# VinAIResearch/Point-Unet

Measured on AMD Instinct MI355X. Metric: points_per_sec_forward, higher is better.
Workload: dtype f32

## Files before the change

### point-unet_amd/csrc/common.h

```cpp
#pragma once

#include <hip/hip_runtime.h>

#include <cstdarg>
#include <cstdint>
#include <cstdio>
#include <cstring>
#include <map>
#include <string>
#include <vector>

#include "../../include/pointseg.h"
#include "../../include/pointseg_train_ops.h"

namespace ps {

void set_error(const char* fmt, ...);

#define PS_HIP(expr)                                                                                  \
    do {                                                                                              \
        hipError_t _e = (expr);                                                                       \
        if (_e != hipSuccess) {                                                                       \
            ps::set_error("%s failed: %s (%s:%d)", #expr, hipGetErrorString(_e), __FILE__, __LINE__); \
            return PS_EHIP;                                                                           \
// ... 91 lines not shown
    int inv_tile = 4096;
    bool gather_reduce_ordered = true;
    int maxpool_bwd_ordered = 1;
    bool train_act_bf16 = true;
    int train_att_gemm_split = -1;
    bool train_att_gemm = true;
    bool train_att128_fwd_gemm = true;
    bool train_fuse_residual = true;
    bool train_merge_syncbn = true;
    int convbn_max_c = 64;
    int convbn_rect_max = 1 << 30;
    bool wgrad_debug = false;
};
void tuning_from_env(Tuning& t);
}

struct ps_context {
    int device = 0;
    ps::Tuning tune;
    hipStream_t own_stream = nullptr;
    hipStream_t stream = nullptr;
    ps::Arena knn_arena;
    ps::Arena net_arena;
    ps::Arena sample_arena;
    ps::DevBuf stage_in;
    ps::DevBuf stage_out;
    ps::DevBuf red_ws;
    ps::DevBuf wgrad_ws;
    ps::PackCache* pack_cache = nullptr;
    ps::DevBuf ops_ring[4];
    int ops_ring_pos = 0;
    bool att_bf16x3 = true;
    bool regchain_b3 = true;
    bool train_b3 = true;
    bool conv_w_transposed = false;
    bool att_df_accum = false;
    const int32_t* walk_order = nullptr;
    int64_t walk_order_n = 0;
    bool pool_bwd_overwrite = false;
    bool train_bf16 = false;
    bool train_act_bf16 = false;
    bool mid_lds_attr = false;
    size_t chain_lds_attr = 48 * 1024;
    std::map<const void*, size_t> regchain_lds_attr;
    bool deferred = false;
    int32_t* h_flags = nullptr;
    unsigned pending_mask = 0;
    uint64_t builds = 0;
    uint64_t samples = 0;
    uint64_t volume_samples = 0;
    uint64_t flag_serial[8] = {};
    int flag_kind[8] = {};
    int flag_slot = 0;
    int sticky_rc = 0;
    std::string sticky_msg;
    hipEvent_t flag_ev[8] = {};
    std::vector<char> host_ring[8];
    int ring_pos = 0;
    std::vector<char>& ring_next() { ring_pos = (ring_pos + 1) & 7; return host_ring[ring_pos]; }
    int check_deferred();
    int check_flag_slot(int s);
    int defer_status(const void* d_words, size_t bytes, int kind, uint64_t serial);
    struct PinSlot { void* p = nullptr; size_t cap = 0; hipEvent_t ev = nullptr; bool busy = false; };
    PinSlot pin[16];
    int pin_pos = 0;
    int upload_async(void* dst, const void* src, size_t bytes);
// ... 69 lines not shown
```

### point-unet_amd/csrc/context.hip

```cpp
#include "common.h"
#include "kdtree_build.h"

#include <cstdlib>

namespace ps {

static thread_local char g_err[512] = "";

void set_error(const char* fmt, ...)
{
    va_list ap;
    va_start(ap, fmt);
    vsnprintf(g_err, sizeof g_err, fmt, ap);
    va_end(ap);
}

int DevBuf::reserve(size_t bytes)
{
    if (bytes <= cap) return PS_OK;
    if (p) {
        hipError_t e = hipDeviceSynchronize();
        if (e != hipSuccess) {
            set_error("hipDeviceSynchronize failed: %s", hipGetErrorString(e));
            return PS_EHIP;
// ... 188 lines not shown
    flag("PS_TRAIN_MERGE_SYNCBN", t.train_merge_syncbn);
    if (num("PS_CONVBN_MAX_C", v) && v >= 0 && v <= 4096) t.convbn_max_c = (int)v;
    if (num("PS_CONVBN_RECT_MAX", v) && v >= 0) t.convbn_rect_max = v > (double)(1 << 30) ? 1 << 30 : (int)v;
    t.wgrad_debug = std::getenv("PS_WGRAD_DEBUG") != nullptr;
#else
    (void)t;
#endif
}
}

extern "C" {
const char* ps_version(void) { return "pointseg-hip 0.1 gfx950"; }
int ps_abi_version(void) { return PS_ABI_VERSION; }

int ps_create(int device, ps_context** out)
{
    PS_CHECK(out != nullptr, "ps_create: out is NULL");
    int count = 0;
    PS_HIP(hipGetDeviceCount(&count));
    PS_CHECK(device >= 0 && device < count, "ps_create: device %d out of range (%d devices)", device, count);
    PS_HIP(hipSetDevice(device));
    ps_context* c = new ps_context();
    c->device = device;
    hipError_t e = hipStreamCreateWithFlags(&c->own_stream, hipStreamNonBlocking);
    if (e != hipSuccess) {
        delete c;
        ps::set_error("hipStreamCreate failed: %s", hipGetErrorString(e));
        return PS_EHIP;
    }
    c->stream = c->own_stream;
    ps::tuning_from_env(c->tune);
#ifdef PS_TUNING_ENV
    if (const char* v = std::getenv("PS_REGCHAIN_B3")) c->regchain_b3 = std::atof(v) != 0;
#endif
    *out = c;
    return PS_OK;
}

int ps_destroy(ps_context* c)
{
    if (!c) return PS_OK;
    (void)hipSetDevice(c->device);
    (void)hipStreamSynchronize(c->stream);
    c->knn_arena.buf.release();
    c->net_arena.buf.release();
    c->sample_arena.buf.release();
    c->stage_in.release();
    c->stage_out.release();
    c->red_ws.release();
    c->wgrad_ws.release();
    for (auto& b : c->ops_ring) b.release();
    if (c->h_flags) (void)hipHostFree(c->h_flags);
    for (auto& e : c->flag_ev)
        if (e) (void)hipEventDestroy(e);
    for (auto& s : c->pin) {
        if (s.p) (void)hipHostFree(s.p);
        if (s.ev) (void)hipEventDestroy(s.ev);
    }
    for (hipEvent_t e : c->event_pool) (void)hipEventDestroy(e);
    if (c->own_stream) (void)hipStreamDestroy(c->own_stream);
    delete c;
    return PS_OK;
}

int ps_set_stream(ps_context* c, void* hip_stream)
{
// ... 95 lines not shown
```

### point-unet_amd/csrc/debug_hooks.h

```cpp
#ifndef POINTSEG_DEBUG_H
#define POINTSEG_DEBUG_H
#include "../../include/pointseg.h"
#ifdef __cplusplus
extern "C" {
#endif
int ps_debug_knn_host(const float* support, const float* queries, int64_t B, int64_t n_support,
                      int64_t n_queries, int64_t K, int32_t* out_idx);
int ps_debug_kdtree_host(const float* support, int64_t n, int32_t* vind, int32_t* nodes, float* pts,
                         int32_t* root_depth, float* bbox);
int ps_debug_kdtree_device(ps_context* ctx, const float* support, int64_t n, int32_t* vind, int32_t* nodes,
                           float* pts, int32_t* root_depth, float* bbox);
#define PS_DEBUG_KDTREE_STATS 22
int ps_debug_kdtree_device_set(ps_context* ctx, const float* support, const int32_t* n, int64_t T, const int32_t* want_copy, int32_t* vind,
                               int32_t* nodes, float* pts, int32_t* fat, int32_t* root_depth, float* bbox, float* copy, int32_t* stats);
int ps_debug_pack_weights(const float* W, int cin, int cout, int ntb, float* out);
int ps_debug_pack_b3(const float* W, int cin, int cout, uint16_t* out);
int ps_debug_gemm32(ps_context* ctx, int split_bf16, const float* x1, int ld1, int c1, const int32_t* g1, const float* x2, int ld2, int c2,
                    const int32_t* g2, int gm, int gn, const float* W, const float* bias, int64_t R, int cout, int leaky, float* y, int ldy);
int ps_debug_gemm32_plan(ps_context* ctx, int split_bf16, int64_t R, int cin, int cout, int* out4);

typedef struct ps_debug_chain_layer {
    const float* W;
    const float* bias;
    int cin, cout, leaky;
    float* y;
    int ldy;
    const float* extra;
    int ld_extra, c_extra;
    const int32_t* extra_gather;
} ps_debug_chain_layer;
typedef struct ps_debug_chain_desc {
    int n_layers;
    ps_debug_chain_layer layer[4];
    const float* x1; const int32_t* g1; int ld1, c1, g1m, g1n;
    const float* x2; const int32_t* g2; int ld2, c2, g2m, g2n;
    int64_t R;
} ps_debug_chain_desc;
int ps_debug_chain(ps_context* ctx, const ps_debug_chain_desc* d, int form);
int ps_debug_chain_plan(const ps_debug_chain_desc* d, int* out4);
int ps_debug_set_regchain_b3(ps_context* ctx, int on);
int ps_debug_att_stage(ps_randla* net, int level, int stage, int form, const float* xyz, const int32_t* idx, const int32_t* order, const float* fg,
                       int64_t n_total, int64_t n_cloud, float* agg);

int ps_debug_set_tuning(ps_context* ctx, const char* field, double value);
int ps_debug_get_tuning(ps_context* ctx, const char* field, double* value);
int ps_debug_tuning_fields(char* buf, int cap);
int ps_debug_volume_sample_args_size(void);

#ifdef __cplusplus
}
#endif
#endif
```

### point-unet_amd/csrc/debug_hooks.hip

```cpp
#include "common.h"

#include <cstring>
#include <vector>
#include "kdtree_build.h"
#include "kdtree_host.h"
#include "rowgemm.h"
#include "attpool.h"
#include "debug_hooks.h"
#include "randla_net.h"

using namespace ps;

extern "C" int ps_debug_volume_sample_args_size(void) { return (int)sizeof(ps_volume_sample_args); }

extern "C" int ps_debug_pack_weights(const float* W, int cin, int cout, int ntb, float* out)
{
    PS_CHECK(W && out && (ntb == 1 || ntb == 2 || ntb == 4), "ps_debug_pack_weights: bad argument");
    pack_weights(W, cin, cout, ntb, out);
    return PS_OK;
}

extern "C" int ps_debug_pack_b3(const float* W, int cin, int cout, uint16_t* out)
{
    PS_CHECK(W && out && cin > 0 && cin % 32 == 0 && cout > 0 && cout % 32 == 0, "ps_debug_pack_b3: bad argument");
// ... 167 lines not shown
            if (regchain_fits(b.steps, b.n, b.s1, b.s2)) rc = regchain(c, b.steps, b.n, b.s1, b.s2, d->R, nullptr);
            else { set_error("ps_debug_chain: not one of regchain's compiled chain shapes"); rc = PS_EINVAL; }
        } else if (form == 2) {
            if (rowchain_lds_plan(b.steps, b.n, b.s1, b.s2, d->R).form == 2) rc = rowchain_lds(c, b.steps, b.n, b.s1, b.s2, d->R);
            else { set_error("ps_debug_chain: the chain does not fit the LDS-staged kernel (channels above %d, mismatched, or a gathered extra)", kChainMaxC); rc = PS_EINVAL; }
        } else {
            RowSrc in1 = b.s1, in2 = b.s2;
            for (int i = 0; i < b.n && rc == PS_OK; ++i) {
                const ChainStep& st = b.steps[i];
                if (i > 0) {
                    in2 = RowSrc();
                    if (st.extra.x) in2 = st.extra;
                }
                float* out = st.y ? st.y : dev + tmp_off[i];
                const int ldo = st.y ? st.ldy : b.L[i].cout;
                rc = rowgemm(c, b.L[i], in1, in2, d->R, out, ldo);
                in1 = RowSrc();
                in1.x = out; in1.ld = ldo; in1.c = b.L[i].cout;
            }
        }
    }
    (void)hipStreamSynchronize(c->stream);
    (void)hipFree(dev);
    return rc;
}

extern "C" int ps_debug_set_regchain_b3(ps_context* c, int on)
{
    PS_CHECK(c && (on == 0 || on == 1), "ps_debug_set_regchain_b3: bad argument");
    c->regchain_b3 = on != 0;
    return PS_OK;
}

extern "C" int ps_debug_att_stage(ps_randla* net, int level, int stage, int form, const float* xyz, const int32_t* idx, const int32_t* order,
                                  const float* fg, int64_t n_total, int64_t n_cloud, float* agg)
{
    PS_CHECK(net && xyz && idx && fg && agg, "ps_debug_att_stage: NULL argument");
    PS_CHECK(net->have_weights, "ps_debug_att_stage: weights not set");
    PS_CHECK(level >= 0 && level < net->cfg.num_layers && (stage == 1 || stage == 2) && form >= 0 && form <= 3, "ps_debug_att_stage: bad level / stage / form");
    PS_CHECK(n_total >= 0 && n_cloud >= 1 && n_total % n_cloud == 0, "ps_debug_att_stage: n_total must be a whole number of clouds");
    ps_context* c = net->ctx;
    PS_HIP(hipSetDevice(c->device));
    const EncLevel& e = net->enc[level];
    const int d = e.d, h = d / 2;
    const bool use_g = d >= 64;
    AttStage s;
    s.xyz = xyz; s.idx = idx; s.order = order; s.fg = fg; s.lfa1 = &e.lfa1; s.agg = agg;
    s.n_total = n_total; s.n_cloud = n_cloud; s.d = d; s.k = net->cfg.k_n; s.ldf = use_g ? h + d : h;
    s.p32 = e.has_p32 ? &e.p32 : nullptr;
    s.lfa2 = stage == 2 ? &e.lfa2 : nullptr;
    s.wbot = use_g ? (stage == 1 ? &e.bot1 : &e.bot2) : nullptr;
    s.wfull = use_g ? nullptr : (stage == 1 ? &e.full1 : &e.full2);
    int rc = PS_EINVAL;
    if (form == 0) rc = att_pool_stage(c, s);
    else if (form == 1 && att_pool32b_fits(s)) rc = att_pool32b_stage(c, s);
    else if (form == 2 && att_pool32_fits(s)) rc = att_pool32_stage(c, s);
    else if (form == 3) rc = att_pool16_stage(c, s);
    else set_error("ps_debug_att_stage: the level (d = %d, %lld rows) does not fit the 32x32 form %d", d, (long long)n_total, form);
    (void)hipStreamSynchronize(c->stream);
    return rc;
}

static bool is_bool(double v) { return v == 0 || v == 1; }
static bool is_int_in(double v, double lo, double hi) { return v >= lo && v <= hi && v == (double)(int64_t)v; }

#define PS_TUNING_FIELDS(X)                                                \
// ... 176 lines not shown
```

### point-unet_amd/csrc/randla.hip

```cpp
#include "attpool.h"
#include "common.h"
#include "randla_net.h"
#include "rowgemm.h"

#include <memory>

namespace ps {

template <int KN>
__global__ __launch_bounds__(256) void pool_max_kernel(const float* __restrict__ feat, const int32_t* __restrict__ idx, const int32_t* __restrict__ order,
                                                       float* __restrict__ out, int rows_out, int m_cloud, int n_cloud, int K, int c4 ,
                                                       unsigned char* __restrict__ ties )
{
    const int per_xcd = (rows_out + 7) >> 3;
    const int xcd = blockIdx.x & 7;
    const size_t lim = (size_t)min(rows_out, (xcd + 1) * per_xcd) * c4;
    for (size_t t = (size_t)xcd * per_xcd * c4 + (size_t)(blockIdx.x >> 3) * 256 + threadIdx.x; t < lim; t += (size_t)(gridDim.x >> 3) * 256) {
        const int r = (int)(t / c4), q = (int)(t - (size_t)r * c4);
        const int row = order ? (r / m_cloud) * m_cloud + order[r] : r;
        const int base = (row / m_cloud) * n_cloud;
        const int32_t* ix = idx + (size_t)row * K;
        const float4* f4 = reinterpret_cast<const float4*>(feat);
        float4 m;
        if constexpr (KN > 0) {
// ... 422 lines not shown
        d_in = 2 * d;
    }

    {
        Stage st(c, "decoder_0", 1);
        PS_TRY(rowgemm(c, net->decoder0, src(X, d_in, d_in), none, B * n[L], dec0, d_in));
    }
    tap(30, dec0, B * n[L] * d_in);

    const float* up = dec0;
    int up_c = d_in;
    for (int j = 0; j < L; ++j) {
        const int lvl = L - 1 - j;
        const float* skip = lvl == 0 ? encb[0] : poolb[lvl - 1];
        const int skip_c = net->dec[j].cout;
        RowSrc s2 = src(up, up_c, up_c);
        s2.gather = pyr->interp_idx[lvl];
        s2.gm = (int)n[lvl];
        s2.gn = (int)n[lvl + 1];
        char nm[48];
        std::snprintf(nm, sizeof nm, "dec%d", j);
        if (j == L - 1) {
            ChainStep ch[4] = {step(net->dec[j], net->keep_taps ? decb[j] : nullptr, skip_c), step(net->fc1, nullptr, 0), step(net->fc2, nullptr, 0),
                               step(net->fc, logits, cfg.num_classes)};
            const RowSrc s1 = src(skip, skip_c, skip_c);
            if (rowchain_fits(ch, 4, s1, s2)) {
                Stage st(c, "head", 1);
                PS_TRY(rowchain(c, ch, 4, s1, s2, B * n[lvl], &net->chains));
                if (net->keep_taps) tap(40 + j, decb[j], B * n[lvl] * skip_c);
                return PS_OK;
            }
        }
        Stage st(c, nm, 1);
        PS_TRY(rowgemm(c, net->dec[j], src(skip, skip_c, skip_c), s2, B * n[lvl], decb[j], skip_c));
        tap(40 + j, decb[j], B * n[lvl] * skip_c);
        up = decb[j];
        up_c = skip_c;
    }
    {
        Stage st(c, "head", 3);
        PS_TRY(rowgemm(c, net->fc1, src(up, up_c, up_c), none, B * n[0], h1, 64));
        PS_TRY(rowgemm(c, net->fc2, src(h1, 64, 64), none, B * n[0], h2, 32));
        PS_TRY(rowgemm(c, net->fc, src(h2, 32, 32), none, B * n[0], logits, cfg.num_classes));
    }
    return PS_OK;
}

extern "C" int ps_randla_keep_taps(ps_randla* net, int on)
{
    PS_CHECK(net, "ps_randla_keep_taps: net is NULL");
    net->keep_taps = on != 0;
    return PS_OK;
}

extern "C" int ps_randla_tap(ps_randla* net, int which, float* host_out, int64_t count)
{
    PS_CHECK(net && host_out, "ps_randla_tap: NULL argument");
    for (auto& t : net->taps)
        if (t.which == which) {
            PS_CHECK(t.count == count, "ps_randla_tap: tensor %d has %lld floats, caller expects %lld", which, (long long)t.count, (long long)count);
            PS_HIP(hipMemcpyAsync(host_out, t.p, sizeof(float) * (size_t)count, hipMemcpyDeviceToHost, net->ctx->stream));
            PS_HIP(hipStreamSynchronize(net->ctx->stream));
            return PS_OK;
        }
    set_error("ps_randla_tap: no tensor %d (run a forward first; the last decoder step's rows are only kept after ps_randla_keep_taps)", which);
    return PS_EINVAL;
}
// ... 1 lines not shown
```

### point-unet_amd/csrc/regchain.hip

```cpp
#include <algorithm>
#include <type_traits>

#include "b3_ops.h"
#include "mfma_tile.h"
#include "rowgemm.h"

namespace ps {

struct RcLayer {
    const float* wp;
    const float* bias;
    float* y;
    const float* ex;
    int ca, cb;
    int ta, tb;
    int cout, ot;
    int ks, ntb;
    int ldy, ldex, leaky;
    int w_off, b_off;
};
struct RcArgs {
    const float* x1; const int32_t* g1; int ld1, g1m, g1n;
    const float* x2; const int32_t* g2; int ld2, g2m, g2n;
    int n, R;
    RcLayer l[kChainMaxSteps];
    const float* image;
    int image_floats;
};

template <int N_, int A0_, int B0_, int O0_, int B1_ = 0, int O1_ = 0, int B2_ = 0, int O2_ = 0, int B3_ = 0, int O3_ = 0>
struct RcShape {
    static constexpr int N = N_, A0 = A0_;
    static constexpr int B[4] = {B0_, B1_, B2_, B3_};
    static constexpr int O[4] = {O0_, O1_, O2_, O3_};
    static constexpr int A(int l) { return l == 0 ? A0_ : O[l - 1]; }
    static constexpr int IN(int l) { return A(l) + B[l]; }
    static constexpr int maxt()
    {
        int m = 1;
        for (int l = 0; l < N_; ++l) {
            m = IN(l) > m ? IN(l) : m;
            m = O[l] > m ? O[l] : m;
        }
        return m;
    }
};

template <int T0, int NT, int MT>
__device__ __forceinline__ void rc_load(float (&dst)[MT][4], const float* __restrict__ rowp, int c, bool vec, int g)
{
#pragma unroll
    for (int t = 0; t < NT; ++t) {
        const int ch = t * 16 + 4 * g;
        if (vec) {
            float4 v = make_float4(0.f, 0.f, 0.f, 0.f);
            if (t + 1 < NT || ch < c) v = *reinterpret_cast<const float4*>(rowp + ch);
            dst[T0 + t][0] = v.x; dst[T0 + t][1] = v.y; dst[T0 + t][2] = v.z; dst[T0 + t][3] = v.w;
        } else {
#pragma unroll
            for (int q = 0; q < 4; ++q) dst[T0 + t][q] = (t + 1 < NT || ch + q < c) ? rowp[ch + q] : 0.f;
        }
    }
}

struct RcF32 {
    static constexpr int kThreads = 256;
    static constexpr int kPairFloats = 256;
    template <int IT, int OT, int MT>
    static __device__ __forceinline__ void mma(f32x4 (&acc)[OT], const float (&act)[MT][4], const float* wl, int lane)
    {
        const float* w = wl + lane;
#pragma unroll
        for (int t0 = 0; t0 < OT; t0 += 4) {
#pragma unroll
            for (int ti = 0; ti < IT; ++ti)
#pragma unroll
                for (int q = 0; q < 4; ++q)
#pragma unroll
                    for (int to = t0; to < (t0 + 4 < OT ? t0 + 4 : OT); ++to)
                        acc[to] = __builtin_amdgcn_mfma_f32_16x16x4f32(w[((to * IT + ti) * 4 + q) * 64], act[ti][q], acc[to], 0, 0, 0);
            if (t0 + 4 < OT) __builtin_amdgcn_sched_barrier(0);
        }
    }
    static __device__ __forceinline__ void stage(const RcLayer& y, float* dst)
    {
        const int it_n = y.ta + y.tb;
        const int ln = threadIdx.x & 63, q = threadIdx.x >> 6;
        const int i = ln & 15, gg = ln >> 4;
        const int npairs = it_n * y.ot;
// ... 50 lines not shown
                    for (int pl = 0; pl < 3; ++pl) a.p[pl] = w[((to * KP + kp) * 3 + pl) * 64];
                    acc[to] = b3_mfma16_6(a, b[kp], acc[to]);
                }
            if (t0 + 4 < OT) __builtin_amdgcn_sched_barrier(0);
        }
    }
    static __device__ __forceinline__ void stage(const RcLayer& y, float* dst)
    {
        const int kp_n = (y.ta + y.tb) / 2;
        uint4* out = reinterpret_cast<uint4*>(dst + y.w_off);
        for (int s = threadIdx.x; s < y.ot * kp_n * 64; s += kThreads) {
            const int ln = s & 63, slot = s >> 6;
            const int to = slot / kp_n, kp = slot - to * kp_n;
            const int i = ln & 15, gg = ln >> 4;
            const int cblk = to / y.ntb, j = to - cblk * y.ntb;
            float v[8];
#pragma unroll
            for (int e = 0; e < 8; ++e) {
                const int ti = 2 * kp + (e >> 2), q = e & 3;
                int k;
                bool kok;
                if (ti < y.ta) { k = ti * 16 + 4 * gg + q; kok = k < y.ca; }
                else { k = (ti - y.ta) * 16 + 4 * gg + q; kok = k < y.cb; k += y.ca; }
                v[e] = 0.f;
                if (kok && to * 16 + i < y.cout) v[e] = y.wp[(((size_t)cblk * y.ks + (k >> 2)) * 64 + ((k & 3) * 16 + i)) * y.ntb + j];
            }
            const B3Planes p = b3_split8<3>(v);
#pragma unroll
            for (int pl = 0; pl < 3; ++pl) out[(slot * 3 + pl) * 64 + ln] = p.p[pl];
        }
    }
};

template <class S, class P, int L>
__device__ __forceinline__ void rc_layer(const RcArgs& a, float (&act)[S::maxt()][4], const float* lds, int lane, int g, int row, int rr, bool ok)
{
    if constexpr (L < S::N) {
        constexpr int IT = S::IN(L), OT = S::O[L], TA = S::A(L), TB = S::B[L];
        const RcLayer& y = a.l[L];
        if constexpr (L > 0 && TB > 0) {
            const bool ve = (y.cb & 3) == 0 && (y.ldex & 3) == 0 && (reinterpret_cast<uintptr_t>(y.ex) & 15) == 0;
            rc_load<TA, TB>(act, y.ex + (size_t)rr * y.ldex, y.cb, ve, g);
        }
        f32x4 acc[OT];
#pragma unroll
        for (int to = 0; to < OT; ++to) acc[to] = f32x4{0.f, 0.f, 0.f, 0.f};
        if constexpr (L > 0) __builtin_amdgcn_sched_barrier(0);
        P::template mma<IT, OT>(acc, act, lds + y.w_off, lane);
        const bool vy = y.y && (y.cout & 3) == 0 && (y.ldy & 3) == 0 && (reinterpret_cast<uintptr_t>(y.y) & 15) == 0;
#pragma unroll
        for (int to = 0; to < OT; ++to) {
            const int ch = to * 16 + 4 * g;
            const float4 b = *reinterpret_cast<const float4*>(lds + y.b_off + ch);
            float v[4] = {acc[to][0] + b.x, acc[to][1] + b.y, acc[to][2] + b.z, acc[to][3] + b.w};
#pragma unroll
            for (int q = 0; q < 4; ++q) {
                if (y.leaky) v[q] = leaky02(v[q]);
                act[to][q] = v[q];
            }
            if (y.y && ok) {
                float* o = y.y + (size_t)row * y.ldy + ch;
                if (vy) {
                    if (to + 1 < OT || ch < y.cout) *reinterpret_cast<float4*>(o) = make_float4(v[0], v[1], v[2], v[3]);
                } else {
#pragma unroll
                    for (int q = 0; q < 4; ++q)
                        if (to + 1 < OT || ch + q < y.cout) o[q] = v[q];
                }
            }
        }
        rc_layer<S, P, L + 1>(a, act, lds, lane, g, row, rr, ok);
    }
}

template <class P>
__device__ __forceinline__ void rc_stage(const RcArgs& a, float* dst)
{
    for (int l = 0; l < a.n; ++l) {
        const RcLayer& y = a.l[l];
        P::stage(y, dst);
        for (int e = threadIdx.x; e < y.ot * 16; e += P::kThreads) dst[y.b_off + e] = e < y.cout ? y.bias[e] : 0.f;
    }
}

template <class P>
__global__ __launch_bounds__(P::kThreads) void rc_pack_kernel(RcArgs a, float* out) { rc_stage<P>(a, out); }

template <class S, class P>
__global__ __launch_bounds__(P::kThreads) void regchain_kernel(RcArgs a)
{
    extern __shared__ __attribute__((aligned(16))) float rc_lds[];
    constexpr int MT = S::maxt(), WAVES = P::kThreads / 64;
    const int wave = threadIdx.x >> 6, lane = threadIdx.x & 63;
    const int p = lane & 15, g = lane >> 4;
    if (a.image) {
        for (int i = threadIdx.x; i < a.image_floats / 4; i += P::kThreads) reinterpret_cast<float4*>(rc_lds)[i] = reinterpret_cast<const float4*>(a.image)[i];
    } else {
        rc_stage<P>(a, rc_lds);
    }
    __syncthreads();

    const bool v1 = (a.l[0].ca & 3) == 0 && (a.ld1 & 3) == 0 && (reinterpret_cast<uintptr_t>(a.x1) & 15) == 0;
    const bool v2 = (a.l[0].cb & 3) == 0 && (a.ld2 & 3) == 0 && (reinterpret_cast<uintptr_t>(a.x2) & 15) == 0;
    const int stride = gridDim.x * WAVES;
    auto load_inputs = [&](int tile, float (&dst)[MT][4]) {
        const int rr = min(tile * 16 + p, a.R - 1);
        const int s1 = a.g1 ? (a.g1m ? (rr / a.g1m) * a.g1n : 0) + a.g1[rr] : rr;
        rc_load<0, S::A0>(dst, a.x1 + (size_t)s1 * a.ld1, a.l[0].ca, v1, g);
        if constexpr (S::B[0] > 0) {
            const int s2 = a.g2 ? (a.g2m ? (rr / a.g2m) * a.g2n : 0) + a.g2[rr] : rr;
            rc_load<S::A0, S::B[0]>(dst, a.x2 + (size_t)s2 * a.ld2, a.l[0].cb, v2, g);
        }
    };
    int tile = blockIdx.x * WAVES + wave;
    float act[MT][4], nxt[MT][4];
    if (tile * 16 < a.R) load_inputs(tile, nxt);
    for (; tile * 16 < a.R; tile += stride) {
#pragma unroll
        for (int t = 0; t < S::IN(0); ++t)
#pragma unroll
            for (int q = 0; q < 4; ++q) act[t][q] = nxt[t][q];
        if ((tile + stride) * 16 < a.R) load_inputs(tile + stride, nxt);
        const int row = tile * 16 + p;
        rc_layer<S, P, 0>(a, act, rc_lds, lane, g, row, min(row, a.R - 1), row < a.R);
    }
}

static inline int rc_tiles(int c) { return (c + 15) / 16; }

using RcFc0 = RcShape<2, 1, 0, 1, 0, 1>;
using RcEnc0 = RcShape<2, 1, 0, 1, 1, 2>;
using RcOne0 = RcShape<1, 1, 0, 1>;
using RcPair1 = RcShape<2, 2, 0, 2, 0, 4>;
using RcPair1b = RcShape<2, 4, 0, 2, 0, 4>;
using RcEnc1 = RcShape<2, 4, 0, 4, 2, 8>;
using RcPair2 = RcShape<2, 8, 0, 4, 0, 8>;
using RcHead = RcShape<4, 2, 2, 2, 0, 4, 0, 2, 0, 1>;

template <class S>
static bool rc_matches(const RcArgs& a)
{
    if (a.n != S::N) return false;
    for (int l = 0; l < S::N; ++l)
        if (a.l[l].ta != S::A(l) || a.l[l].tb != S::B[l] || a.l[l].ot != S::O[l]) return false;
    return true;
}

template <class S>
constexpr bool rc_even_inputs()
{
    for (int l = 0; l < S::N; ++l)
        if (S::IN(l) & 1) return false;
    return true;
}
template <class S>
constexpr bool kRcSplit = std::is_same<S, RcHead>::value || std::is_same<S, RcEnc1>::value || std::is_same<S, RcPair1>::value ||
                          std::is_same<S, RcPair1b>::value;

static size_t rc_layout(RcArgs& a, int pair_floats)
{
    int off = 0;
    for (int i = 0; i < a.n; ++i) {
        RcLayer& y = a.l[i];
        y.w_off = off; off += y.ot * (y.ta + y.tb) * pair_floats;
        y.b_off = off; off += y.ot * 16;
    }
    return (size_t)off * sizeof(float);
}

static bool rc_build(const ChainStep* steps, int n_steps, const RowSrc& s1, const RowSrc& s2, RcArgs& a, size_t& lds_bytes)
{
    if (n_steps < 1 || n_steps > kChainMaxSteps) return false;
    a = RcArgs{};
    a.x1 = s1.x; a.g1 = s1.gather; a.ld1 = s1.ld; a.g1m = s1.gm; a.g1n = s1.gn;
    a.x2 = s2.x; a.g2 = s2.gather; a.ld2 = s2.ld; a.g2m = s2.gm; a.g2n = s2.gn;
    a.n = n_steps;
    int prev = 0;
    for (int i = 0; i < n_steps; ++i) {
        const PackedLinear* L = steps[i].L;
        if (!L || !L->wp || !L->bias) return false;
        if (steps[i].extra.x && (i == 0 || steps[i].extra.gather)) return false;
        RcLayer& y = a.l[i];
        y.wp = L->wp; y.bias = L->bias; y.y = steps[i].y; y.ldy = steps[i].ldy;
        y.ex = i > 0 ? steps[i].extra.x : nullptr; y.ldex = steps[i].extra.ld;
        y.ca = i == 0 ? s1.c : prev;
        y.cb = i == 0 ? s2.c : (steps[i].extra.x ? steps[i].extra.c : 0);
        if (y.ca + y.cb != L->cin) return false;
        y.ta = rc_tiles(y.ca); y.tb = rc_tiles(y.cb);
        y.cout = L->cout; y.ot = rc_tiles(L->cout);
        y.ks = L->ks; y.ntb = L->ntb; y.leaky = L->leaky;
        prev = L->cout;
    }
    lds_bytes = rc_layout(a, RcF32::kPairFloats);
    return rc_matches<RcFc0>(a) || rc_matches<RcEnc0>(a) || rc_matches<RcOne0>(a) || rc_matches<RcPair1>(a) || rc_matches<RcPair1b>(a) ||
           rc_matches<RcEnc1>(a) || rc_matches<RcPair2>(a) || rc_matches<RcHead>(a);
}

bool regchain_fits(const ChainStep* steps, int n_steps, const RowSrc& s1, const RowSrc& s2)
{
    RcArgs a;
    size_t lds = 0;
    return rc_build(steps, n_steps, s1, s2, a, lds);
}

static int rc_blocks(int64_t R, size_t lds_bytes, int waves)
{
    const int64_t tiles = (R + 15) / 16;
    const int per_cu = std::max(1, std::min(16 / waves, (int)(160 * 1024 / std::max<size_t>(lds_bytes, 1))));
    return (int)std::max<int64_t>(1, std::min<int64_t>((tiles + waves - 1) / waves, 256 * per_cu));
}

ChainPlan regchain_plan(const ChainStep* steps, int n_steps, const RowSrc& s1, const RowSrc& s2, int64_t R)
{
    ChainPlan p;
    RcArgs a;
    if (!rc_build(steps, n_steps, s1, s2, a, p.lds_bytes)) return ChainPlan();
    p.form = 1;
    p.blocks = rc_blocks(R, p.lds_bytes, RcF32::kThreads / 64);
    return p;
}

template <class S, class P>
static int rc_run(ps_context* c, RcArgs& a, ChainCache* cache)
{
    constexpr bool split = std::is_same<P, RcB3>::value;
    const size_t lds_bytes = rc_layout(a, P::kPairFloats);
    if (cache) {
        ChainCache::Entry* hit = nullptr;
        for (auto& e : cache->entries)
            if (e.wp0 == a.l[0].wp && e.wp_last == a.l[a.n - 1].wp && e.n == a.n && e.ca == a.l[0].ca && e.cb == a.l[0].cb && e.split == split) hit = &e;
        if (!hit) {
            cache->entries.emplace_back();
            hit = &cache->entries.back();
            hit->wp0 = a.l[0].wp; hit->wp_last = a.l[a.n - 1].wp; hit->n = a.n; hit->ca = a.l[0].ca; hit->cb = a.l[0].cb; hit->split = split;
            PS_TRY(hit->img.reserve(lds_bytes));
            hipLaunchKernelGGL(rc_pack_kernel<P>, dim3(1), dim3(P::kThreads), 0, c->stream, a, hit->img.as<float>());
            PS_HIP(hipGetLastError());
        }
        a.image = hit->img.as<float>();
        a.image_floats = (int)(lds_bytes / sizeof(float));
    }
    size_t& have = c->regchain_lds_attr[reinterpret_cast<const void*>(regchain_kernel<S, P>)];
    if (lds_bytes > 48 * 1024 && lds_bytes > have) {
        PS_HIP(hipFuncSetAttribute(reinterpret_cast<const void*>(regchain_kernel<S, P>), hipFuncAttributeMaxDynamicSharedMemorySize, (int)lds_bytes));
        have = lds_bytes;
    }
    hipLaunchKernelGGL((regchain_kernel<S, P>), dim3(rc_blocks(a.R, lds_bytes, P::kThreads / 64)), dim3(P::kThreads), lds_bytes, c->stream, a);
    PS_HIP(hipGetLastError());
    return PS_OK;
}

template <class S>
static int rc_route(ps_context* c, RcArgs& a, ChainCache* cache)
{
    if constexpr (kRcSplit<S>) {
        static_assert(rc_even_inputs<S>(), "the split-bf16 policy takes its K axis in pairs of 16-channel tiles");
        if (c->regchain_b3) return rc_run<S, RcB3>(c, a, cache);
    }
    return rc_run<S, RcF32>(c, a, cache);
}

int regchain(ps_context* c, const ChainStep* steps, int n_steps, const RowSrc& s1, const RowSrc& s2, int64_t R, ChainCache* cache)
{
    if (R <= 0) return PS_OK;
    RcArgs a;
    size_t lds_bytes = 0;
    PS_CHECK(rc_build(steps, n_steps, s1, s2, a, lds_bytes), "regchain: not one of the compiled chain shapes");
    PS_CHECK(R < (int64_t)1 << 31, "regchain: too many rows");
    a.R = (int)R;
    if (rc_matches<RcFc0>(a)) return rc_route<RcFc0>(c, a, cache);
    if (rc_matches<RcEnc0>(a)) return rc_route<RcEnc0>(c, a, cache);
    if (rc_matches<RcOne0>(a)) return rc_route<RcOne0>(c, a, cache);
    if (rc_matches<RcPair1>(a)) return rc_route<RcPair1>(c, a, cache);
    if (rc_matches<RcPair1b>(a)) return rc_route<RcPair1b>(c, a, cache);
    if (rc_matches<RcEnc1>(a)) return rc_route<RcEnc1>(c, a, cache);
    if (rc_matches<RcPair2>(a)) return rc_route<RcPair2>(c, a, cache);
    return rc_route<RcHead>(c, a, cache);
}

}
```

### point-unet_amd/csrc/rowgemm.h

```cpp
#pragma once

#include <vector>

#include "common.h"

namespace ps {

struct PackedLinear {
    const float* wp = nullptr;
    const float* wq = nullptr;
    const void* wb = nullptr;
    const float* w32 = nullptr;
    const void* w32b = nullptr;
    const float* bias = nullptr;
    int cin = 0, cout = 0;
    int ks = 0;
    int ntb = 0;
    int cblocks = 0;
    int leaky = 0;
    int accum = 0;
    size_t packed_floats() const { return (size_t)cblocks * ks * 64 * ntb; }
    int nchunks() const { return (cin + 63) / 64; }
    size_t kperm_floats() const { return (size_t)cblocks * nchunks() * 16 * 64 * ntb; }
    size_t bf16_bytes() const { return (size_t)cblocks * nchunks() * 2 * 64 * ntb * 16; }
// ... 17 lines not shown
    int rw = 1, cw = 1, sk = 1, pd = 2;
    int rgroups = 0, cgroups = 0;
};
Gemm32Plan gemm32_plan(const Tuning& tn, int64_t R, int cin, int cout);
Gemm32Plan gemm32b_plan(const Tuning& tn, int64_t R, int cin, int cout);
bool gemm32_fits(const PackedLinear& L, const RowSrc& s1, const RowSrc& s2, int64_t R, int ldy);
int gemm32(ps_context* c, const PackedLinear& L, const RowSrc& s1, const RowSrc& s2, int64_t R, float* y, int ldy);
void pack_p32b(const float* W, int cin, int cout, uint16_t* out);
bool gemm32b_fits(const PackedLinear& L, const RowSrc& s1, const RowSrc& s2, int64_t R, int ldy);
int gemm32b(ps_context* c, const PackedLinear& L, const RowSrc& s1, const RowSrc& s2, int64_t R, float* y, int ldy);

int rowgemm(ps_context* c, const PackedLinear& L, const RowSrc& s1, const RowSrc& s2, int64_t R, float* y, int ldy);

constexpr int kChainMaxC = 96;
constexpr int kChainMaxSteps = 4;
struct ChainStep {
    const PackedLinear* L = nullptr;
    float* y = nullptr;
    int ldy = 0;
    RowSrc extra;
};
bool rowchain_fits(const ChainStep* steps, int n_steps, const RowSrc& s1, const RowSrc& s2);
bool regchain_fits(const ChainStep* steps, int n_steps, const RowSrc& s1, const RowSrc& s2);
struct ChainCache {
    struct Entry { const float* wp0 = nullptr; const float* wp_last = nullptr; int n = 0, ca = 0, cb = 0; bool split = false; DevBuf img; };
    std::vector<Entry> entries;
    void clear()
    {
        for (auto& e : entries) e.img.release();
        entries.clear();
    }
};
int regchain(ps_context* c, const ChainStep* steps, int n_steps, const RowSrc& s1, const RowSrc& s2, int64_t R, ChainCache* cache);
int rowchain_lds(ps_context* c, const ChainStep* steps, int n_steps, const RowSrc& s1, const RowSrc& s2, int64_t R);
struct ChainPlan {
    int form = 0;
    int blocks = 0;
    size_t lds_bytes = 0;
    int fast_in = 0;
};
ChainPlan regchain_plan(const ChainStep* steps, int n_steps, const RowSrc& s1, const RowSrc& s2, int64_t R);
ChainPlan rowchain_lds_plan(const ChainStep* steps, int n_steps, const RowSrc& s1, const RowSrc& s2, int64_t R);
ChainPlan rowchain_plan(const ChainStep* steps, int n_steps, const RowSrc& s1, const RowSrc& s2, int64_t R);
int rowchain(ps_context* c, const ChainStep* steps, int n_steps, const RowSrc& s1, const RowSrc& s2, int64_t R, ChainCache* cache = nullptr);

bool gemm_b3_fits(const Tuning& tn, int64_t R, int64_t K, int64_t N, const float* x, int64_t ldx, bool one_plane);
size_t gemm_b3_plane_bytes(int64_t K, int64_t N);
int gemm_b3(ps_context* c, const float* x, int64_t ldx, const float* w, int64_t sk, int64_t sn, const float* bias, int64_t R, int64_t K, int64_t N, int leaky,
            int accumulate, float* y, int64_t ldy, void* planes, int pack = 1);

}
```

Baseline: 192.6 million.

## Specialize register-chain kernels on compile-time layer facts and route decoder layer

Adds compile-time 'facts' template parameters (leaky mask, store mask, partial-tile mask, vectorized last store) to the register-chain kernel. When runtime arguments match a known configuration, the host launches a variant with no alignment checks or bounds guards, and full tiles are split from a single tail tile. It also adds a one-layer decoder chain shape so the non-final decoder linear layers run through the register-chain path instead of rowgemm. This costs more kernel instantiations and adds dispatch logic that must match the runtime facts exactly.

```diff
diff --git a/point-unet_amd/csrc/common.h b/point-unet_amd/csrc/common.h
--- a/point-unet_amd/csrc/common.h
+++ b/point-unet_amd/csrc/common.h
@@ -147,6 +147,7 @@
     int ops_ring_pos = 0;
     bool att_bf16x3 = true;
     bool regchain_b3 = true;
+    bool regchain_special = true;
     bool train_b3 = true;
     bool conv_w_transposed = false;
     bool att_df_accum = false;
diff --git a/point-unet_amd/csrc/context.hip b/point-unet_amd/csrc/context.hip
--- a/point-unet_amd/csrc/context.hip
+++ b/point-unet_amd/csrc/context.hip
@@ -244,6 +244,7 @@
     ps::tuning_from_env(c->tune);
 #ifdef PS_TUNING_ENV
     if (const char* v = std::getenv("PS_REGCHAIN_B3")) c->regchain_b3 = std::atof(v) != 0;
+    if (const char* v = std::getenv("PS_REGCHAIN_SPECIAL")) c->regchain_special = std::atof(v) != 0;
 #endif
     *out = c;
     return PS_OK;
diff --git a/point-unet_amd/csrc/debug_hooks.h b/point-unet_amd/csrc/debug_hooks.h
--- a/point-unet_amd/csrc/debug_hooks.h
+++ b/point-unet_amd/csrc/debug_hooks.h
@@ -39,6 +39,8 @@
 int ps_debug_chain(ps_context* ctx, const ps_debug_chain_desc* d, int form);
 int ps_debug_chain_plan(const ps_debug_chain_desc* d, int* out4);
 int ps_debug_set_regchain_b3(ps_context* ctx, int on);
+int ps_debug_set_regchain_special(ps_context* ctx, int on);
+int ps_debug_regchain_facts(ps_context* ctx, const ps_debug_chain_desc* d, int* out);
 int ps_debug_att_stage(ps_randla* net, int level, int stage, int form, const float* xyz, const int32_t* idx, const int32_t* order, const float* fg,
                        int64_t n_total, int64_t n_cloud, float* agg);
 
diff --git a/point-unet_amd/csrc/debug_hooks.hip b/point-unet_amd/csrc/debug_hooks.hip
--- a/point-unet_amd/csrc/debug_hooks.hip
+++ b/point-unet_amd/csrc/debug_hooks.hip
@@ -223,6 +223,23 @@
     return PS_OK;
 }
 
+extern "C" int ps_debug_set_regchain_special(ps_context* c, int on)
+{
+    PS_CHECK(c && (on == 0 || on == 1), "ps_debug_set_regchain_special: bad argument");
+    c->regchain_special = on != 0;
+    return PS_OK;
+}
+
+extern "C" int ps_debug_regchain_facts(ps_context* c, const ps_debug_chain_desc* d, int* out)
+{
+    PS_CHECK(c && d && out && d->R >= 1, "ps_debug_regchain_facts: bad argument");
+    static const float nothing = 0.f;
+    ChainBuild b;
+    PS_TRY(chain_describe(d, b, &nothing));
+    out[0] = regchain_special_fits(c, b.steps, b.n, b.s1, b.s2, d->R) ? 1 : 0;
+    return PS_OK;
+}
+
 extern "C" int ps_debug_att_stage(ps_randla* net, int level, int stage, int form, const float* xyz, const int32_t* idx, const int32_t* order,
                                   const float* fg, int64_t n_total, int64_t n_cloud, float* agg)
 {
diff --git a/point-unet_amd/csrc/randla.hip b/point-unet_amd/csrc/randla.hip
--- a/point-unet_amd/csrc/randla.hip
+++ b/point-unet_amd/csrc/randla.hip
@@ -478,7 +478,12 @@
             }
         }
         Stage st(c, nm, 1);
-        PS_TRY(rowgemm(c, net->dec[j], src(skip, skip_c, skip_c), s2, B * n[lvl], decb[j], skip_c));
+        ChainStep one[1] = {step(net->dec[j], decb[j], skip_c)};
+        if (j < L - 1 && regchain_fits(one, 1, src(skip, skip_c, skip_c), s2)) {
+            PS_TRY(rowchain(c, one, 1, src(skip, skip_c, skip_c), s2, B * n[lvl], &net->chains));
+        } else {
+            PS_TRY(rowgemm(c, net->dec[j], src(skip, skip_c, skip_c), s2, B * n[lvl], decb[j], skip_c));
+        }
         tap(40 + j, decb[j], B * n[lvl] * skip_c);
         up = decb[j];
         up_c = skip_c;
diff --git a/point-unet_amd/csrc/regchain.hip b/point-unet_amd/csrc/regchain.hip
--- a/point-unet_amd/csrc/regchain.hip
+++ b/point-unet_amd/csrc/regchain.hip
@@ -46,15 +46,27 @@
     }
 };
 
-template <int T0, int NT, int MT>
+struct RcAny {
+    static constexpr bool kAny = true;
+    static constexpr unsigned kLeaky = 0, kStore = 0, kPart = 0;
+    static constexpr bool kVecLast = false;
+};
+template <unsigned LEAKY, unsigned STORE, unsigned PART, bool VEC_LAST>
+struct RcFacts {
+    static constexpr bool kAny = false;
+    static constexpr unsigned kLeaky = LEAKY, kStore = STORE, kPart = PART;
+    static constexpr bool kVecLast = VEC_LAST;
+};
+
+template <int T0, int NT, int MT, int MODE = 0>
 __device__ __forceinline__ void rc_load(float (&dst)[MT][4], const float* __restrict__ rowp, int c, bool vec, int g)
 {
 #pragma unroll
     for (int t = 0; t < NT; ++t) {
         const int ch = t * 16 + 4 * g;
-        if (vec) {
+        if (MODE != 0 || vec) {
             float4 v = make_float4(0.f, 0.f, 0.f, 0.f);
-            if (t + 1 < NT || ch < c) v = *reinterpret_cast<const float4*>(rowp + ch);
+            if (MODE == 2 || t + 1 < NT || ch < c) v = *reinterpret_cast<const float4*>(rowp + ch);
             dst[T0 + t][0] = v.x; dst[T0 + t][1] = v.y; dst[T0 + t][2] = v.z; dst[T0 + t][3] = v.w;
         } else {
 #pragma unroll
@@ -171,22 +183,30 @@
     }
 };
 
-template <class S, class P, int L>
+template <class S, class P, class F, int L, bool TAIL>
 __device__ __forceinline__ void rc_layer(const RcArgs& a, float (&act)[S::maxt()][4], const float* lds, int lane, int g, int row, int rr, bool ok)
 {
     if constexpr (L < S::N) {
         constexpr int IT = S::IN(L), OT = S::O[L], TA = S::A(L), TB = S::B[L];
         const RcLayer& y = a.l[L];
         if constexpr (L > 0 && TB > 0) {
-            const bool ve = (y.cb & 3) == 0 && (y.ldex & 3) == 0 && (reinterpret_cast<uintptr_t>(y.ex) & 15) == 0;
-            rc_load<TA, TB>(act, y.ex + (size_t)rr * y.ldex, y.cb, ve, g);
+            if constexpr (F::kAny) {
+                const bool ve = (y.cb & 3) == 0 && (y.ldex & 3) == 0 && (reinterpret_cast<uintptr_t>(y.ex) & 15) == 0;
+                rc_load<TA, TB>(act, y.ex + (size_t)rr * y.ldex, y.cb, ve, g);
+            } else {
+                rc_load<TA, TB, S::maxt(), (F::kPart >> (4 + L) & 1) ? 1 : 2>(act, y.ex + (size_t)rr * y.ldex, y.cb, true, g);
+            }
         }
         f32x4 acc[OT];
 #pragma unroll
         for (int to = 0; to < OT; ++to) acc[to] = f32x4{0.f, 0.f, 0.f, 0.f};
         if constexpr (L > 0) __builtin_amdgcn_sched_barrier(0);
         P::template mma<IT, OT>(acc, act, lds + y.w_off, lane);
-        const bool vy = y.y && (y.cout & 3) == 0 && (y.ldy & 3) == 0 && (reinterpret_cast<uintptr_t>(y.y) & 15) == 0;
+        constexpr bool kSpec = !F::kAny, kStored = (F::kStore >> L & 1) != 0, kWhole = kSpec && !(F::kPart >> L & 1);
+        constexpr bool kVecStore = L + 1 < S::N || F::kVecLast;
+        const bool leaky = kSpec ? (F::kLeaky >> L & 1) != 0 : y.leaky != 0;
+        const bool stored = kSpec ? kStored && (!TAIL || ok) : y.y && ok;
+        const bool vy = kSpec ? kVecStore : y.y && (y.cout & 3) == 0 && (y.ldy & 3) == 0 && (reinterpret_cast<uintptr_t>(y.y) & 15) == 0;
 #pragma unroll
         for (int to = 0; to < OT; ++to) {
             const int ch = to * 16 + 4 * g;
@@ -194,21 +214,21 @@
             float v[4] = {acc[to][0] + b.x, acc[to][1] + b.y, acc[to][2] + b.z, acc[to][3] + b.w};
 #pragma unroll
             for (int q = 0; q < 4; ++q) {
-                if (y.leaky) v[q] = leaky02(v[q]);
+                if (leaky) v[q] = leaky02(v[q]);
                 act[to][q] = v[q];
             }
-            if (y.y && ok) {
+            if (stored) {
                 float* o = y.y + (size_t)row * y.ldy + ch;
                 if (vy) {
-                    if (to + 1 < OT || ch < y.cout) *reinterpret_cast<float4*>(o) = make_float4(v[0], v[1], v[2], v[3]);
+                    if (kWhole || to + 1 < OT || ch < y.cout) *reinterpret_cast<float4*>(o) = make_float4(v[0], v[1], v[2], v[3]);
                 } else {
 #pragma unroll
                     for (int q = 0; q < 4; ++q)
-                        if (to + 1 < OT || ch + q < y.cout) o[q] = v[q];
+                        if (kWhole || to + 1 < OT || ch + q < y.cout) o[q] = v[q];
                 }
             }
         }
-        rc_layer<S, P, L + 1>(a, act, lds, lane, g, row, rr, ok);
+        rc_layer<S, P, F, L + 1, TAIL>(a, act, lds, lane, g, row, rr, ok);
     }
 }
 
@@ -225,7 +245,7 @@
 template <class P>
 __global__ __launch_bounds__(P::kThreads) void rc_pack_kernel(RcArgs a, float* out) { rc_stage<P>(a, out); }
 
-template <class S, class P>
+template <class S, class P, class F = RcAny>
 __global__ __launch_bounds__(P::kThreads) void regchain_kernel(RcArgs a)
 {
     extern __shared__ __attribute__((aligned(16))) float rc_lds[];
@@ -239,29 +259,62 @@
     }
     __syncthreads();
 
-    const bool v1 = (a.l[0].ca & 3) == 0 && (a.ld1 & 3) == 0 && (reinterpret_cast<uintptr_t>(a.x1) & 15) == 0;
-    const bool v2 = (a.l[0].cb & 3) == 0 && (a.ld2 & 3) == 0 && (reinterpret_cast<uintptr_t>(a.x2) & 15) == 0;
     const int stride = gridDim.x * WAVES;
-    auto load_inputs = [&](int tile, float (&dst)[MT][4]) {
-        const int rr = min(tile * 16 + p, a.R - 1);
-        const int s1 = a.g1 ? (a.g1m ? (rr / a.g1m) * a.g1n : 0) + a.g1[rr] : rr;
-        rc_load<0, S::A0>(dst, a.x1 + (size_t)s1 * a.ld1, a.l[0].ca, v1, g);
-        if constexpr (S::B[0] > 0) {
-            const int s2 = a.g2 ? (a.g2m ? (rr / a.g2m) * a.g2n : 0) + a.g2[rr] : rr;
-            rc_load<S::A0, S::B[0]>(dst, a.x2 + (size_t)s2 * a.ld2, a.l[0].cb, v2, g);
-        }
-    };
     int tile = blockIdx.x * WAVES + wave;
     float act[MT][4], nxt[MT][4];
-    if (tile * 16 < a.R) load_inputs(tile, nxt);
-    for (; tile * 16 < a.R; tile += stride) {
+    auto take_next = [&]() {
 #pragma unroll
         for (int t = 0; t < S::IN(0); ++t)
 #pragma unroll
             for (int q = 0; q < 4; ++q) act[t][q] = nxt[t][q];
-        if ((tile + stride) * 16 < a.R) load_inputs(tile + stride, nxt);
-        const int row = tile * 16 + p;
-        rc_layer<S, P, 0>(a, act, rc_lds, lane, g, row, min(row, a.R - 1), row < a.R);
+    };
+    if constexpr (F::kAny) {
+        const bool v1 = (a.l[0].ca & 3) == 0 && (a.ld1 & 3) == 0 && (reinterpret_cast<uintptr_t>(a.x1) & 15) == 0;
+        const bool v2 = (a.l[0].cb & 3) == 0 && (a.ld2 & 3) == 0 && (reinterpret_cast<uintptr_t>(a.x2) & 15) == 0;
+        auto load_inputs = [&](int tile, float (&dst)[MT][4]) {
+            const int rr = min(tile * 16 + p, a.R - 1);
+            const int s1 = a.g1 ? (a.g1m ? (rr / a.g1m) * a.g1n : 0) + a.g1[rr] : rr;
+            rc_load<0, S::A0>(dst, a.x1 + (size_t)s1 * a.ld1, a.l[0].ca, v1, g);
+            if constexpr (S::B[0] > 0) {
+                const int s2 = a.g2 ? (a.g2m ? (rr / a.g2m) * a.g2n : 0) + a.g2[rr] : rr;
+                rc_load<S::A0, S::B[0]>(dst, a.x2 + (size_t)s2 * a.ld2, a.l[0].cb, v2, g);
+            }
+        };
+        if (tile * 16 < a.R) load_inputs(tile, nxt);
+        for (; tile * 16 < a.R; tile += stride) {
+            take_next();
+            if ((tile + stride) * 16 < a.R) load_inputs(tile + stride, nxt);
+            const int row = tile * 16 + p;
+            rc_layer<S, P, F, 0, true>(a, act, rc_lds, lane, g, row, min(row, a.R - 1), row < a.R);
+        }
+    } else {
+        const int full = a.R >> 4;
+        auto load_inputs = [&](int tile, float (&dst)[MT][4], auto partial) {
+            const int r0 = tile * 16 + p;
+            const int rr = decltype(partial)::value ? min(r0, a.R - 1) : r0;
+            const int s1 = a.g1 ? a.g1[rr] : rr;
+            rc_load<0, S::A0, MT, 2>(dst, a.x1 + (size_t)s1 * a.ld1, a.l[0].ca, true, g);
+            if constexpr (S::B[0] > 0) {
+                const int s2 = a.g2 ? a.g2[rr] : rr;
+                rc_load<S::A0, S::B[0], MT, 2>(dst, a.x2 + (size_t)s2 * a.ld2, a.l[0].cb, true, g);
+            }
+        };
+        auto prefetch = [&](int t) {
+            if (t < full) load_inputs(t, nxt, std::false_type());
+            else if (t * 16 < a.R) load_inputs(t, nxt, std::true_type());
+        };
+        prefetch(tile);
+        for (; tile < full; tile += stride) {
+            take_next();
+            prefetch(tile + stride);
+            const int row = tile * 16 + p;
+            rc_layer<S, P, F, 0, false>(a, act, rc_lds, lane, g, row, row, true);
+        }
+        if (tile * 16 < a.R) {
+            take_next();
+            const int row = tile * 16 + p;
+            rc_layer<S, P, F, 0, true>(a, act, rc_lds, lane, g, row, min(row, a.R - 1), row < a.R);
+        }
     }
 }
 
@@ -275,6 +328,7 @@
 using RcEnc1 = RcShape<2, 4, 0, 4, 2, 8>;
 using RcPair2 = RcShape<2, 8, 0, 4, 0, 8>;
 using RcHead = RcShape<4, 2, 2, 2, 0, 4, 0, 2, 0, 1>;
+using RcDec1 = RcShape<1, 2, 8, 2>;
 
 template <class S>
 static bool rc_matches(const RcArgs& a)
@@ -286,6 +340,80 @@
 }
 
 template <class S>
+struct RcTag { using type = S; };
+template <class Fn>
+static auto rc_with_shape(const RcArgs& a, Fn&& fn)
+{
+    if (rc_matches<RcFc0>(a)) return fn(RcTag<RcFc0>());
+    if (rc_matches<RcEnc0>(a)) return fn(RcTag<RcEnc0>());
+    if (rc_matches<RcOne0>(a)) return fn(RcTag<RcOne0>());
+    if (rc_matches<RcPair1>(a)) return fn(RcTag<RcPair1>());
+    if (rc_matches<RcPair1b>(a)) return fn(RcTag<RcPair1b>());
+    if (rc_matches<RcEnc1>(a)) return fn(RcTag<RcEnc1>());
+    if (rc_matches<RcPair2>(a)) return fn(RcTag<RcPair2>());
+    if (rc_matches<RcDec1>(a)) return fn(RcTag<RcDec1>());
+    return fn(RcTag<RcHead>());
+}
+
+struct RcFactBits {
+    bool ok = false;
+    unsigned leaky = 0, store = 0, part = 0;
+    bool vec_last = true;
+};
+static bool rc_vec(const void* p, int c, int ld) { return (c & 3) == 0 && (ld & 3) == 0 && (reinterpret_cast<uintptr_t>(p) & 15) == 0; }
+
+static void rc_single_cloud(RcArgs& a)
+{
+    if (!a.g1 || a.R <= a.g1m) a.g1m = a.g1n = 0;
+    if (!a.g2 || a.R <= a.g2m) a.g2m = a.g2n = 0;
+}
+
+static RcFactBits rc_facts(const RcArgs& a)
+{
+    RcFactBits f;
+    const RcLayer& y0 = a.l[0];
+    f.ok = a.g1m == 0 && a.g2m == 0 && rc_vec(a.x1, y0.ca, a.ld1) && y0.ca % 16 == 0 && (y0.tb == 0 || (rc_vec(a.x2, y0.cb, a.ld2) && y0.cb % 16 == 0));
+    for (int l = 0; l < a.n; ++l) {
+        const RcLayer& y = a.l[l];
+        if (y.leaky) f.leaky |= 1u << l;
+        if (y.cout % 16) f.part |= 1u << l;
+        if (l > 0 && y.tb > 0) {
+            if (y.cb % 16) f.part |= 16u << l;
+            f.ok = f.ok && rc_vec(y.ex, y.cb, y.ldex);
+        }
+        if (y.y) {
+            f.store |= 1u << l;
+            const bool v = rc_vec(y.y, y.cout, y.ldy);
+            if (l + 1 < a.n) f.ok = f.ok && v;
+            else f.vec_last = v;
+        }
+    }
+    return f;
+}
+template <class F>
+static bool rc_facts_match(const RcFactBits& f)
+{
+    return f.ok && f.leaky == F::kLeaky && f.store == F::kStore && f.part == F::kPart && f.vec_last == F::kVecLast;
+}
+
+template <class... Fs>
+struct RcList {};
+template <class S>
+struct RcSpecs { using type = RcList<>; };
+template <> struct RcSpecs<RcOne0> { using type = RcList<RcFacts<0b1, 0b1, 0b1, true>>; };
+template <> struct RcSpecs<RcEnc0> { using type = RcList<RcFacts<0b11, 0b10, 16u << 1, true>>; };
+template <> struct RcSpecs<RcPair1> { using type = RcList<RcFacts<0b01, 0b11, 0, true>>; };
+template <> struct RcSpecs<RcPair1b> { using type = RcList<RcFacts<0b01, 0b11, 0, true>>; };
+template <> struct RcSpecs<RcEnc1> { using type = RcList<RcFacts<0b11, 0b10, 0, true>>; };
+template <> struct RcSpecs<RcPair2> { using type = RcList<RcFacts<0b01, 0b11, 0, true>>; };
+template <> struct RcSpecs<RcDec1> { using type = RcList<RcFacts<0b1, 0b1, 0, true>>; };
+template <> struct RcSpecs<RcHead> { using type = RcList<RcFacts<0b0111, 0b1000, 0b1000, true>, RcFacts<0b0111, 0b1000, 0b1000, false>>; };
+
+static bool rc_any_match(const RcFactBits&, RcList<>) { return false; }
+template <class F, class... Fs>
+static bool rc_any_match(const RcFactBits& f, RcList<F, Fs...>) { return rc_facts_match<F>(f) || rc_any_match(f, RcList<Fs...>()); }
+
+template <class S>
 constexpr bool rc_even_inputs()
 {
     for (int l = 0; l < S::N; ++l)
@@ -295,6 +423,8 @@
 template <class S>
 constexpr bool kRcSplit = std::is_same<S, RcHead>::value || std::is_same<S, RcEnc1>::value || std::is_same<S, RcPair1>::value ||
                           std::is_same<S, RcPair1b>::value;
+template <class S>
+using RcRouted = typename std::conditional<kRcSplit<S>, RcB3, RcF32>::type;
 
 static size_t rc_layout(RcArgs& a, int pair_floats)
 {
@@ -332,7 +462,7 @@
     }
     lds_bytes = rc_layout(a, RcF32::kPairFloats);
     return rc_matches<RcFc0>(a) || rc_matches<RcEnc0>(a) || rc_matches<RcOne0>(a) || rc_matches<RcPair1>(a) || rc_matches<RcPair1b>(a) ||
-           rc_matches<RcEnc1>(a) || rc_matches<RcPair2>(a) || rc_matches<RcHead>(a);
+           rc_matches<RcEnc1>(a) || rc_matches<RcPair2>(a) || rc_matches<RcDec1>(a) || rc_matches<RcHead>(a);
 }
 
 bool regchain_fits(const ChainStep* steps, int n_steps, const RowSrc& s1, const RowSrc& s2)
@@ -359,7 +489,7 @@
     return p;
 }
 
-template <class S, class P>
+template <class S, class P, class F = RcAny>
 static int rc_run(ps_context* c, RcArgs& a, ChainCache* cache)
 {
     constexpr bool split = std::is_same<P, RcB3>::value;
@@ -379,19 +509,36 @@
         a.image = hit->img.as<float>();
         a.image_floats = (int)(lds_bytes / sizeof(float));
     }
-    size_t& have = c->regchain_lds_attr[reinterpret_cast<const void*>(regchain_kernel<S, P>)];
+    size_t& have = c->regchain_lds_attr[reinterpret_cast<const void*>(regchain_kernel<S, P, F>)];
     if (lds_bytes > 48 * 1024 && lds_bytes > have) {
-        PS_HIP(hipFuncSetAttribute(reinterpret_cast<const void*>(regchain_kernel<S, P>), hipFuncAttributeMaxDynamicSharedMemorySize, (int)lds_bytes));
+        PS_HIP(hipFuncSetAttribute(reinterpret_cast<const void*>(regchain_kernel<S, P, F>), hipFuncAttributeMaxDynamicSharedMemorySize, (int)lds_bytes));
         have = lds_bytes;
     }
-    hipLaunchKernelGGL((regchain_kernel<S, P>), dim3(rc_blocks(a.R, lds_bytes, P::kThreads / 64)), dim3(P::kThreads), lds_bytes, c->stream, a);
+    hipLaunchKernelGGL((regchain_kernel<S, P, F>), dim3(rc_blocks(a.R, lds_bytes, P::kThreads / 64)), dim3(P::kThreads), lds_bytes, c->stream, a);
     PS_HIP(hipGetLastError());
     return PS_OK;
 }
 
+template <class S, class P>
+static int rc_run_special(ps_context* c, RcArgs& a, ChainCache* cache, const RcFactBits&, RcList<>) { return rc_run<S, P>(c, a, cache); }
+template <class S, class P, class F, class... Fs>
+static int rc_run_special(ps_context* c, RcArgs& a, ChainCache* cache, const RcFactBits& f, RcList<F, Fs...>)
+{
+    if (rc_facts_match<F>(f)) return rc_run<S, P, F>(c, a, cache);
+    return rc_run_special<S, P>(c, a, cache, f, RcList<Fs...>());
+}
+
+template <class S>
+static bool rc_takes_special(const ps_context* c, const RcArgs& a)
+{
+    if (!c->regchain_special || (kRcSplit<S> && !c->regchain_b3)) return false;
+    return rc_any_match(rc_facts(a), typename RcSpecs<S>::type());
+}
+
 template <class S>
 static int rc_route(ps_context* c, RcArgs& a, ChainCache* cache)
 {
+    if (rc_takes_special<S>(c, a)) return rc_run_special<S, RcRouted<S>>(c, a, cache, rc_facts(a), typename RcSpecs<S>::type());
     if constexpr (kRcSplit<S>) {
         static_assert(rc_even_inputs<S>(), "the split-bf16 policy takes its K axis in pairs of 16-channel tiles");
         if (c->regchain_b3) return rc_run<S, RcB3>(c, a, cache);
@@ -407,14 +554,18 @@
     PS_CHECK(rc_build(steps, n_steps, s1, s2, a, lds_bytes), "regchain: not one of the compiled chain shapes");
     PS_CHECK(R < (int64_t)1 << 31, "regchain: too many rows");
     a.R = (int)R;
-    if (rc_matches<RcFc0>(a)) return rc_route<RcFc0>(c, a, cache);
-    if (rc_matches<RcEnc0>(a)) return rc_route<RcEnc0>(c, a, cache);
-    if (rc_matches<RcOne0>(a)) return rc_route<RcOne0>(c, a, cache);
-    if (rc_matches<RcPair1>(a)) return rc_route<RcPair1>(c, a, cache);
-    if (rc_matches<RcPair1b>(a)) return rc_route<RcPair1b>(c, a, cache);
-    if (rc_matches<RcEnc1>(a)) return rc_route<RcEnc1>(c, a, cache);
-    if (rc_matches<RcPair2>(a)) return rc_route<RcPair2>(c, a, cache);
-    return rc_route<RcHead>(c, a, cache);
-}
-
-}
+    rc_single_cloud(a);
+    return rc_with_shape(a, [&](auto tag) { return rc_route<typename decltype(tag)::type>(c, a, cache); });
+}
+
+bool regchain_special_fits(const ps_context* c, const ChainStep* steps, int n_steps, const RowSrc& s1, const RowSrc& s2, int64_t R)
+{
+    RcArgs a;
+    size_t lds_bytes = 0;
+    if (R <= 0 || R >= (int64_t)1 << 31 || !rc_build(steps, n_steps, s1, s2, a, lds_bytes)) return false;
+    a.R = (int)R;
+    rc_single_cloud(a);
+    return rc_with_shape(a, [&](auto tag) { return rc_takes_special<typename decltype(tag)::type>(c, a); });
+}
+
+}
diff --git a/point-unet_amd/csrc/rowgemm.h b/point-unet_amd/csrc/rowgemm.h
--- a/point-unet_amd/csrc/rowgemm.h
+++ b/point-unet_amd/csrc/rowgemm.h
@@ -73,6 +73,7 @@
     }
 };
 int regchain(ps_context* c, const ChainStep* steps, int n_steps, const RowSrc& s1, const RowSrc& s2, int64_t R, ChainCache* cache);
+bool regchain_special_fits(const ps_context* c, const ChainStep* steps, int n_steps, const RowSrc& s1, const RowSrc& s2, int64_t R);
 int rowchain_lds(ps_context* c, const ChainStep* steps, int n_steps, const RowSrc& s1, const RowSrc& s2, int64_t R);
 struct ChainPlan {
     int form = 0;
```

After: 192.0 million (median of 2 runs). No clear change (-0.3%).
